# LMCache/LMCache

Hardware: NVIDIA H100
Metric: kv_encode_decode_raw_GBps (higher is better)
Workload: dtype f32->u8 (bf16 KV)

## Files before the change

lmcache_b200/csrc/ac_core.cuh:

```cuda
#pragma once
#include <stdint.h>

#if defined(__CUDACC__)
#define B2_HD __host__ __device__ __forceinline__
#else
#define B2_HD inline
#endif

namespace b200kv {

constexpr int kLp = 33;
constexpr int kMaxSym = 31;
constexpr int kGroup = 256;

B2_HD uint32_t f2u(float f) {
#if defined(__CUDA_ARCH__)
    return __float_as_uint(f);
#else
    union { float f; uint32_t u; } v; v.f = f; return v.u;
#endif
}
B2_HD float u2f(uint32_t u) {
#if defined(__CUDA_ARCH__)
    return __uint_as_float(u);
// ... 599 lines not shown
    const int64_t NL = 2 * (int64_t)L;
    lo.ngroups = (t + kGroup - 1) / kGroup;
    lo.off_cdf = 64;
    if (compact) {
        lo.off_maxes = align16(lo.off_cdf + NL);
        lo.off_lengths = align16(lo.off_maxes + NL * t * 2);
        lo.off_payload = align16(lo.off_lengths + (int64_t)lo.ngroups * NL * C);
    } else {
        lo.off_maxes = align16(lo.off_cdf + NL * C * kLp * 2);
        lo.off_lengths = align16(lo.off_maxes + NL * t * 2);
        lo.off_payload = align16(lo.off_lengths + (int64_t)lo.ngroups * NL * C * 4);
    }
    return lo;
}

constexpr int kHdrMax = 36;
B2_HD int hdr_mask_bytes(int nb) { return (nb + 7) >> 3; }
B2_HD uint32_t hdr_len(uint32_t mask, int nb) {
#if defined(__CUDA_ARCH__)
    const uint32_t nz = (uint32_t)__popc(mask);
#else
    uint32_t nz = 0;
    for (uint32_t m = mask; m; m &= m - 1u) ++nz;
#endif
    const uint32_t h = (uint32_t)hdr_mask_bytes(nb) + (nz ? nz - 1u : 0u);
    return h + (h & 1u);
}
inline uint32_t hdr_write_host(uint8_t* dst, const uint32_t* cnt, int nb) {
    uint32_t mask = 0;
    for (int i = 0; i < nb; ++i) mask |= (cnt[i] ? 1u : 0u) << i;
// ... 12 lines not shown
```

lmcache_b200/csrc/codec.cu:

```cuda
#include <cuda_bf16.h>
#include <cuda_fp16.h>
#include <cuda_runtime.h>
#include <stdint.h>
#include <stdlib.h>
#include <string.h>

#include "ac_core.cuh"
#include "common.cuh"

namespace b200kv {

constexpr int CT = 128;
constexpr int SPW = 6;
constexpr int SYMW = 43;
constexpr int PAIRW = 33;
constexpr int TEMPW_FUSED = 40;
constexpr int TEMPW_SPLIT = 132;
constexpr int TEMPW_FUSED_RANS = 48;
constexpr int CODER_AC = 0, CODER_RANS = 1;
constexpr int CODER_RANS_COMPACT = 2;
constexpr int kHdrRowWords = 8;
constexpr int TEMPW_FUSED_RANS_HDR = TEMPW_FUSED_RANS + kHdrRowWords;

struct EncParams {
// ... 11 lines not shown
    uint64_t* sizes_out;
    uint32_t* temp;
    uint32_t* rstate;
    uint32_t* tile_tot;
    unsigned long long* totals;
    unsigned int* err;
    int32_t lb, nlay;
    uint8_t* arena;
    int64_t arena_bytes;
    unsigned long long* chunk_base;
    unsigned long long* cursor;
    unsigned int* fail_from;
    unsigned long long* ptotal;
    int64_t* seg;
    int32_t layers_left;
};

__device__ __forceinline__ int launch_plane(const EncParams& P, int local) {
    return local + (local < P.nlay ? P.lb : P.L - P.nlay + P.lb);
}

template <class Prm>
__device__ __forceinline__ Layout layout_of(const Prm& P, int t) {
    return make_layout(P.L, P.C, t, P.compact);
}

__device__ __forceinline__ uint32_t load_len(const uint8_t* sec, int64_t idx, bool compact) {
    return compact ? 2u * (uint32_t)sec[idx] : (uint32_t)reinterpret_cast<const int32_t*>(sec)[idx];
}
__device__ __forceinline__ void store_len(uint8_t* sec, int64_t idx, uint32_t len, bool compact) {
    if (compact) sec[idx] = (uint8_t)(len >> 1);
// ... 36 lines not shown
    if (nb > 16) m |= (uint32_t)*reinterpret_cast<const uint16_t*>(p + 2) << 16;
    if (nb <= 8) m &= 0xffu;
    return nb >= 32 ? m : m & ((1u << nb) - 1u);
}

__device__ __forceinline__ int chunk_tokens_of(const EncParams& P, int j) {
    return j == P.n_chunks - 1 ? P.last_chunk_tokens : P.chunk_tokens;
}

template <bool PAGED>
__device__ __forceinline__ int64_t tok_row(const int64_t* slot_map, int64_t tok) {
    if constexpr (PAGED) return __ldg(slot_map + tok);
    else return tok;
}

template <bool VEC, bool PAGED>
__global__ void __launch_bounds__(256) absmax_kernel(EncParams P, int64_t total_tokens) {
    const int64_t warp = (blockIdx.x * (int64_t)blockDim.x + threadIdx.x) >> 5;
    const int lane = threadIdx.x & 31;
    const int64_t nrows = (int64_t)2 * P.nlay * total_tokens;
    if (warp >= nrows) return;
    const int nl = launch_plane(P, (int)(warp / total_tokens));
    const int64_t T = warp % total_tokens;
    const uint16_t* row = P.pt.p[nl] + tok_row<PAGED>(P.slot_map, P.tok_begin + T) * P.sT;
    uint32_t m = 0;
    if (VEC) {
        const int vec_per_head = P.D >> 3;
        const int nvec = P.H * vec_per_head;
        for (int v = lane; v < nvec; v += 32) {
            const int h = v / vec_per_head, dv = v - h * vec_per_head;
            const uint4 q = __ldg(reinterpret_cast<const uint4*>(row + (int64_t)h * P.sH + dv * 8));
            const uint32_t w[4] = {q.x, q.y, q.z, q.w};
#pragma unroll
            for (int k = 0; k < 4; ++k) {
                const uint32_t a = w[k] & 0x7fff7fffu;
                m = max(m, max(a & 0xffffu, a >> 16));
            }
        }
    } else {
        for (int c = lane; c < P.C; c += 32) {
            const int h = c / P.D, d = c - h * P.D;
            m = max(m, (uint32_t)(__ldg(row + (int64_t)h * P.sH + d) & 0x7fffu));
        }
    }
    m = __reduce_max_sync(0xffffffffu, m);
    if (lane == 0) {
        const int j = (int)(T / P.chunk_tokens);
        const int tj = chunk_tokens_of(P, j);
        const Layout lo = layout_of(P, tj);
        uint16_t* maxes = reinterpret_cast<uint16_t*>(P.out + (int64_t)j * P.out_stride + lo.off_maxes);
        maxes[(int64_t)nl * tj + (T - (int64_t)j * P.chunk_tokens)] = (uint16_t)m;
    }
}

__device__ __forceinline__ uint32_t block_excl_scan(uint32_t v, uint32_t* s_warp, uint32_t* total) {
    const int lane = threadIdx.x & 31, wid = threadIdx.x >> 5;
    uint32_t inc = v;
#pragma unroll
    for (int o = 1; o < 32; o <<= 1) {
        uint32_t n = __shfl_up_sync(0xffffffffu, inc, o);
        if (lane >= o) inc += n;
    }
    if (lane == 31) s_warp[wid] = inc;
    __syncthreads();
    uint32_t base = 0, tot = 0;
#pragma unroll
// ... 107 lines not shown
    x = a + start;
    if (r >= freq) x += m;
}

template <bool FUSED, int DT, bool PAGED, int CODER>
__global__ void __launch_bounds__(CT, FUSED ? 7 : 4) encode_kernel(EncParams P) {
    extern __shared__ __align__(128) uint32_t smem[];
    constexpr int ROWS_W = FUSED ? CT * SYMW : 0;
    constexpr int TAB_W = FUSED ? (CT * kLp * 2 + 3) / 4 : CT * PAIRW;
    uint32_t* rows = smem;
    uint32_t* tab = smem + ROWS_W;
    float* fac = reinterpret_cast<float*>(smem + ((ROWS_W + TAB_W + 3) & ~3));
    __shared__ uint32_t s_warp[CT / 32];

    const int tid = threadIdx.x;
    TileId id;
    if (!decode_tile(P, blockIdx.x, &id)) return;
    const int NL = 2 * P.L;
    const int j = id.j, nl = id.nl, ct = id.ct, t = id.t, gt = id.gt;
    const int c = ct * CT + tid;
    const bool active = c < P.C;
    const int ncols = min(CT, P.C - ct * CT);

    uint8_t* cont = P.out + (int64_t)j * P.out_stride;
    const Layout lo = layout_of(P, t);
    const uint16_t* maxes = reinterpret_cast<const uint16_t*>(cont + lo.off_maxes) + (int64_t)nl * t + id.tok0;
    const float maxq = P.pt.maxq[nl];
    const int64_t s1 = P.sT;
    for (int i = tid; i < gt; i += CT)
        fac[i] = FUSED ? quant_factor_safe(maxq, half_to_float(maxes[i], DT)) : quant_factor(maxq, half_to_float(maxes[i], DT));
    if (FUSED) for (int i = gt + tid; i < kGroup + 8; i += CT) fac[i] = 0.0f;

    const int h = active ? c / P.D : 0;
    const int64_t tokabs = P.tok_begin + (int64_t)j * P.chunk_tokens + id.tok0;
    const uint16_t* cbase = P.pt.p[nl] + (int64_t)h * P.sH + (active ? c - h * P.D : 0);
    const uint16_t* src = cbase + (PAGED ? 0 : tokabs * P.sT);
    uint32_t* trow = P.temp + ((int64_t)blockIdx.x * CT + tid) * P.tempw;
    uint32_t cap = (uint32_t)P.tempw;
    asm volatile("" : "+l"(trow), "+r"(cap));
    uint32_t len = 0u, hlen = 0u;

    if (FUSED) {
        uint32_t* myrow = rows + tid * SYMW;
        uint16_t* cdfr = reinterpret_cast<uint16_t*>(tab);
        uint16_t* crow = cdfr + tid * kLp;
        uint16_t* hist = crow;
#pragma unroll
        for (int i = 0; i < kLp; ++i) crow[i] = 0;
        if (!PAGED) {
            const int lines_per_tok = (ncols * 2 + 127) >> 7;
            const uint16_t* tile0 = P.pt.p[nl] + (P.tok_begin + (int64_t)j * P.chunk_tokens + id.tok0) * P.sT +
                                    (int64_t)((ct * CT) / P.D) * P.sH + ((ct * CT) % P.D);
            if ((ct * CT) / P.D == (ct * CT + ncols - 1) / P.D)
                for (int i = tid; i < gt * lines_per_tok; i += CT) {
                    const int tok = i / lines_per_tok, ln = i - tok * lines_per_tok;
                    asm volatile("prefetch.global.L2 [%0];" ::"l"(tile0 + (int64_t)tok * s1 + ln * 64));
                }
        }
        __syncthreads();
        if (active) {
            constexpr int NB = 2, BT = NB * SPW;
            const int nbatch = (gt + BT - 1) / BT;
            uint16_t xa[BT], xb[BT];
            const uint32_t s1u = (uint32_t)s1;
            const uint32_t two = 2u * (uint32_t)min(P.n_chunks, 1);
            auto load = [&](uint16_t (&x)[BT], int b) {
                const int tk = b * BT;
                if constexpr (PAGED) {
                    const int64_t* sm = P.slot_map + tokabs + tk;
#pragma unroll
                    for (int k = 0; k < BT; ++k) x[k] = tk + k < gt ? __ldg(cbase + __ldg(sm + k) * s1) : (uint16_t)0;
                } else {
                    const uint16_t* q = src + (int64_t)tk * s1;
// ... 55 lines not shown
            uint32_t mask = 0u;
#pragma unroll
            for (int i = 0; i < 32; ++i) mask |= (cnt[i] != 0u ? 1u : 0u) << i;
            const uint32_t wany = __reduce_or_sync(__activemask(), mask);
            CdfAccum2 acc;
            acc.init();
#pragma unroll
            for (uint32_t i = 0; i < 32u; ++i) {
                crow[i] = (uint16_t)acc.value(i);
                if ((wany >> i) & 1u) acc.absorb(fac[cnt[i]]);
            }
            crow[32] = (uint16_t)acc.value(32u);
            if (P.compact) {
                uint32_t w0, w1;
                hlen = build_stream_header(cnt, mask, wany, 2 * ((int)maxq + 1), trow, w0, w1);
                reinterpret_cast<uint2*>(P.rstate)[((int64_t)blockIdx.x * CT + tid) * 2] = make_uint2(w0, w1);
            }
        }
        __syncthreads();
        if (!P.compact) {
            uint16_t* dstc = reinterpret_cast<uint16_t*>(cont + lo.off_cdf) + ((int64_t)nl * P.C + ct * CT) * kLp;
            for (int e = tid; e < ncols * kLp; e += CT) dstc[e] = cdfr[e];
        }
        if (active && CODER == CODER_RANS) {
            uint32_t x = kRansLow;
            const uint16_t* const wend = reinterpret_cast<const uint16_t*>(trow) + 2 * P.tempw;
            int32_t nk = 0;
            const char* const cb = reinterpret_cast<const char*>(crow);
            auto code = [&](uint32_t word, int k) {
                const uint32_t o = (k == 0 ? word << 1 : word >> (5 * k - 1)) & 62u;
                const uint32_t c_lo = *reinterpret_cast<const uint16_t*>(cb + o);
                const uint32_t c_hi = *reinterpret_cast<const uint16_t*>(cb + o + 2);
                rans_put(x, nk, wend, c_lo, c_hi - c_lo);
            };
            int w = (gt - 1) / SPW;
            {
                const uint32_t word = myrow[w];
                for (int k = gt - 1 - w * SPW; k >= 0; --k) code(word, k);
            }
            for (--w; w >= 0; --w) {
                const uint32_t word = myrow[w];
#pragma unroll
                for (int k = SPW - 1; k >= 0; --k) code(word, k);
            }
            if (P.compact) reinterpret_cast<uint2*>(P.rstate)[((int64_t)blockIdx.x * CT + tid) * 2 + 1] = make_uint2(x, hlen);
            else P.rstate[(int64_t)blockIdx.x * CT + tid] = x;
            len = hlen + 4u - 2u * (uint32_t)nk;
        } else if (active) {
            EncState2 st;
            st.init();
            int tk = 0;
            for (int w = 0; tk < gt; ++w) {
                const uint32_t word = myrow[w];
                if (tk + SPW <= gt) {
#pragma unroll
                    for (int k = 0; k < SPW; ++k) {
                        const uint32_t sidx = (word >> (5 * k)) & 31u;
                        const uint32_t c_lo = crow[sidx];
                        enc_symbol2(st, c_lo, (uint32_t)crow[sidx + 1u] - c_lo, trow, cap);
                    }
                    tk += SPW;
// ... 19 lines not shown
#pragma unroll
            for (int i = 0; i < kLp; ++i) cv[i] = prow[i] & 0xffffu;
#pragma unroll
            for (int i = 0; i < 32; ++i) {
                const uint32_t hi = (i == 31) ? 0x10000u : cv[i + 1];
                prow[i] = cv[i] | ((hi - cv[i]) << 16);
            }
            if (CODER == CODER_RANS) {
                uint32_t x = kRansLow;
                const uint16_t* const wend = reinterpret_cast<const uint16_t*>(trow) + 2 * TEMPW_SPLIT;
                int32_t nk = 0;
                for_each_symbol_rev<DT, PAGED, 4>(cbase, P.slot_map, tokabs, s1, gt, fac, maxq, [&](uint32_t q) {
                    const uint32_t pr = prow[q];
                    rans_put(x, nk, wend, pr & 0xffffu, pr >> 16);
                });
                P.rstate[(int64_t)blockIdx.x * CT + tid] = x;
                len = 4u - 2u * (uint32_t)nk;
            } else {
                EncState2 st;
                st.init();
                for_each_symbol<DT, PAGED, 4>(cbase, P.slot_map, tokabs, s1, gt, fac, maxq, [&](uint32_t q) {
                    const uint32_t pr = prow[q];
                    enc_symbol2(st, pr & 0xffffu, pr >> 16, trow, cap);
                });
                len = enc_finish2(st, trow, cap);
                if (st.w > cap) atomicOr(&P.err[j], 1u);
            }
        }
    }

    if (active) store_len(cont + lo.off_lengths, ((int64_t)id.g * NL + nl) * P.C + c, len, P.compact != 0);
    uint32_t tile_total;
    (void)block_excl_scan(len, s_warp, &tile_total);
    if (tid == 0) P.tile_tot[(int64_t)j * P.tiles_full + id.tile_in_chunk] = tile_total;
}

template <int DT, bool PAGED>
__global__ void __launch_bounds__(CT) cdf_kernel(EncParams P) {
    extern __shared__ __align__(128) uint32_t smem[];
    uint32_t* cnts = smem;
    float* fac = reinterpret_cast<float*>(cnts + CT * PAIRW);
    const int tid = threadIdx.x;
    const int NL = 2 * P.L;
    const uint32_t per_chunk = (uint32_t)NL * P.tpp;
    const uint32_t j = blockIdx.x / per_chunk;
    const uint32_t rem = blockIdx.x - j * per_chunk;
    const int nl = (int)(rem / P.tpp);
    const int ct = (int)(rem - (uint32_t)nl * P.tpp);
    const int t = chunk_tokens_of(P, (int)j);
// ... 824 lines not shown
        }
        cudaEventRecord(g_prof_ev[slot][0], stream);
    }
    ~ProfScope() {
        if (!g_prof_on) return;
        cudaEventRecord(g_prof_ev[slot][1], stream);
        g_prof_have[slot] = true;
    }
};

static int enc_tempw(bool fused, int coder, bool compact = false) {
    if (compact) return TEMPW_FUSED_RANS_HDR;
    return fused ? (coder == CODER_RANS ? TEMPW_FUSED_RANS : TEMPW_FUSED) : TEMPW_SPLIT;
}

static size_t enc_ws_layout(int64_t n_tiles_alloc, int n_chunks, int tempw, int coder, bool compact, size_t* off_tot,
                            size_t* off_totals, size_t* off_err, size_t* off_state, size_t* off_temp) {
    size_t o = 0;
    *off_tot = o;    o += (size_t)n_tiles_alloc * 4;  o = (o + 255) & ~(size_t)255;
    *off_totals = o; o += (size_t)n_chunks * 8;       o = (o + 255) & ~(size_t)255;
    *off_err = o;    o += (size_t)n_chunks * 4;       o = (o + 255) & ~(size_t)255;
    *off_state = o;  o += coder == CODER_RANS ? (size_t)n_tiles_alloc * CT * (compact ? 16 : 4) : 0;  o = (o + 255) & ~(size_t)255;
    *off_temp = o;   o += (size_t)n_tiles_alloc * CT * (size_t)tempw * 4;
    return (o + 255) & ~(size_t)255;
}

struct EnclWs { size_t err, ptotal, cbase, state, tot, totals, rstate, temp, bytes; };
static EnclWs encl_ws_layout(int n_chunks, int64_t call_tiles) {
    EnclWs w;
    size_t o = 0;
    auto take = [&](size_t* off, size_t n) { *off = o; o = (o + n + 255) & ~(size_t)255; };
    take(&w.err, (size_t)n_chunks * 4);
    take(&w.ptotal, (size_t)n_chunks * 8);
    take(&w.cbase, (size_t)n_chunks * 8);
    take(&w.state, 16);
    take(&w.tot, (size_t)call_tiles * 4);
    take(&w.totals, (size_t)n_chunks * 8);
    take(&w.rstate, (size_t)call_tiles * CT * 16);
    take(&w.temp, (size_t)call_tiles * CT * TEMPW_FUSED_RANS_HDR * 4);
    w.bytes = o;
    return w;
}

constexpr uint32_t kEncPlanMagic = 0x4e4c5045u;
struct EncPlan {
    uint32_t magic;
    int32_t max_layers;
    uint64_t done;
    EncParams P;
};
static_assert(sizeof(EncPlan) <= sizeof(b200kv_encode_plan_t), "b200kv_encode_plan_t too small");

constexpr size_t kSmemFused = (size_t)(((CT * SYMW + (CT * kLp * 2 + 3) / 4 + 3) & ~3) + kGroup + 8) * 4;
constexpr int kStageRans = 12 * 1024;

static int launch_absmax(const EncParams& P, const b200kv_kv_desc* kv, int64_t total_tokens, cudaStream_t stream) {
    bool vec = (kv->D % 8 == 0) && (kv->sT % 8 == 0) && (kv->sH % 8 == 0);
    for (int nl = 0; nl < 2 * P.L && vec; ++nl) vec = (reinterpret_cast<uintptr_t>(P.pt.p[nl]) & 15) == 0;
    const bool paged = P.slot_map != nullptr;
    const int64_t rows = 2 * (int64_t)P.nlay * total_tokens;
    const int64_t blocks = (rows + 7) / 8;
    B2_REQUIRE(blocks < (1ll << 31), "too many rows in one call");
    if (vec && !paged) absmax_kernel<true, false><<<(unsigned)blocks, 256, 0, stream>>>(P, total_tokens);
    else if (vec) absmax_kernel<true, true><<<(unsigned)blocks, 256, 0, stream>>>(P, total_tokens);
    else if (!paged) absmax_kernel<false, false><<<(unsigned)blocks, 256, 0, stream>>>(P, total_tokens);
    else absmax_kernel<false, true><<<(unsigned)blocks, 256, 0, stream>>>(P, total_tokens);
    B2_CHECK_CUDA(cudaGetLastError());
    return 0;
}

static size_t dec_ws_layout(int64_t tiles_max, int n_chunks, size_t* off_tb) {
    size_t o = ((size_t)n_chunks * sizeof(DecChunk) + 255) & ~(size_t)255;
    *off_tb = o;
// ... 69 lines not shown
                                                                                      stride, out);
    B2_CHECK_CUDA(cudaGetLastError());
    return 0;
}

int64_t b200kv_encode_workspace_bytes(int32_t L, int32_t H, int32_t D, int32_t chunk_tokens, int32_t n_chunks,
                                      int32_t coder) {
    if (L <= 0 || H <= 0 || D <= 0 || chunk_tokens <= 0 || n_chunks <= 0) return -2;
    coder &= 0xff;
    const bool compact = coder == CODER_RANS_COMPACT;
    if (compact) coder = CODER_RANS;
    if (coder != CODER_AC && coder != CODER_RANS) return -2;
    if (compact && chunk_tokens > kGroup) return -2;
    const int64_t G = (chunk_tokens + kGroup - 1) / kGroup;
    const int64_t n_tiles = (int64_t)n_chunks * G * 2 * L * tiles_per_plane(H * D);
    size_t a, b, c, d, e;
    return (int64_t)enc_ws_layout(n_tiles, n_chunks, enc_tempw(chunk_tokens <= kGroup, coder, compact), coder, compact, &a, &b, &c, &d, &e);
}

int64_t b200kv_decode_workspace_bytes(int32_t L, int32_t H, int32_t D, int32_t chunk_tokens, int32_t n_chunks) {
    if (L <= 0 || H <= 0 || D <= 0 || chunk_tokens <= 0 || n_chunks <= 0) return -2;
    const int64_t G = (chunk_tokens + kGroup - 1) / kGroup;
    const int64_t tiles_max = G * 2 * L * tiles_per_plane(H * D);
    size_t a;
    return (int64_t)dec_ws_layout(tiles_max, n_chunks, &a);
}

int b200kv_encode_chunks(const b200kv_kv_desc* kv, int64_t tok_begin, int32_t n_chunks, int32_t chunk_tokens,
                         int32_t last_chunk_tokens, const float* key_bins, const float* value_bins, int32_t coder,
                         void* out, int64_t out_stride, uint64_t* sizes_out, void* workspace, int64_t workspace_bytes,
                         void* stream_) {
    cudaStream_t stream = static_cast<cudaStream_t>(stream_);
// ... 12 lines not shown
    B2_REQUIRE(out != nullptr && (reinterpret_cast<uintptr_t>(out) & 15) == 0 && (out_stride & 15) == 0,
               "out / out_stride must be 16-byte aligned");
    B2_REQUIRE(tok_begin >= 0, "tok_begin must be >= 0");
    P.sT = kv->sT; P.sH = kv->sH; P.tok_begin = tok_begin;
    P.slot_map = kv->slot_map;
    const bool paged = kv->slot_map != nullptr;
    P.L = kv->L; P.H = kv->H; P.D = kv->D; P.C = kv->H * kv->D; P.dtype = kv->dtype;
    P.n_chunks = n_chunks; P.chunk_tokens = chunk_tokens; P.last_chunk_tokens = last_chunk_tokens;
    P.tpp = tiles_per_plane(P.C);
    P.out = static_cast<uint8_t*>(out);
    P.out_stride = out_stride;
    P.sizes_out = sizes_out;
    P.lb = 0; P.nlay = P.L;
    P.arena = nullptr; P.arena_bytes = 0; P.chunk_base = nullptr; P.cursor = nullptr; P.fail_from = nullptr;
    P.ptotal = nullptr; P.seg = nullptr; P.layers_left = 0;
    const Layout lo = make_layout(P.L, P.C, chunk_tokens, P.compact);
    B2_REQUIRE(out_stride >= lo.off_payload + 16, "out_stride smaller than the fixed container sections");

    const int64_t G = lo.ngroups;
    const int64_t per_group = 2 * (int64_t)P.L * P.tpp;
    const int64_t tiles_full = G * per_group;
    const int64_t n_tiles = (int64_t)n_chunks * tiles_full;
    const bool fused = chunk_tokens <= kGroup;
    P.tiles_full = (int32_t)tiles_full;
    P.tempw = enc_tempw(fused, coder, P.compact != 0);
    size_t off_tot, off_totals, off_err, off_state, off_temp;
    const size_t need = enc_ws_layout(n_tiles, n_chunks, P.tempw, coder, P.compact != 0, &off_tot, &off_totals, &off_err, &off_state,
                                      &off_temp);
    B2_REQUIRE(workspace != nullptr && workspace_bytes >= (int64_t)need, "workspace too small");
    B2_REQUIRE(n_tiles < (1ll << 31) && tiles_full < (1ll << 31), "too many tiles in one call");
    uint8_t* ws = static_cast<uint8_t*>(workspace);
    P.tile_tot = reinterpret_cast<uint32_t*>(ws + off_tot);
    P.totals = reinterpret_cast<unsigned long long*>(ws + off_totals);
    P.err = reinterpret_cast<unsigned int*>(ws + off_err);
    P.temp = reinterpret_cast<uint32_t*>(ws + off_temp);
    P.rstate = reinterpret_cast<uint32_t*>(ws + off_state);
    B2_CHECK_CUDA(cudaMemsetAsync(ws, 0, off_state, stream));

    const int64_t total_tokens = (int64_t)(n_chunks - 1) * chunk_tokens + last_chunk_tokens;
    for (int i = 0; i <= kProfFinalize; ++i) g_prof_have[i] = false;
    {
        ProfScope prof(kProfAbsmax, stream);
        if (int rc = launch_absmax(P, kv, total_tokens, stream)) return rc;
    }
    const size_t smem_fused = kSmemFused;
    const size_t smem_split = (size_t)(((CT * PAIRW + 3) & ~3) + kGroup + 4) * 4;
    const size_t smem_cdf = (size_t)(CT * PAIRW + kGroup) * 4;
#define B2_LAUNCH_ENC1(FUSED, DT, PAGED, CODER, SMEM)                                                      \
    do {                                                                                                   \
        B2_CHECK_CUDA(cudaFuncSetAttribute(encode_kernel<FUSED, DT, PAGED, CODER>,                         \
                                           cudaFuncAttributeMaxDynamicSharedMemorySize, (int)(SMEM)));     \
        encode_kernel<FUSED, DT, PAGED, CODER><<<(unsigned)n_tiles, CT, (SMEM), stream>>>(P);              \
    } while (0)
#define B2_LAUNCH_ENC(FUSED, DT, PAGED, SMEM)                                                              \
    do {                                                                                                   \
        if (coder == CODER_RANS) B2_LAUNCH_ENC1(FUSED, DT, PAGED, CODER_RANS, SMEM);                       \
        else B2_LAUNCH_ENC1(FUSED, DT, PAGED, CODER_AC, SMEM);                                             \
    } while (0)
#define B2_LAUNCH_ENC2(FUSED, SMEM)                                                                        \
    do {                                                                                                   \
        if (P.dtype == B200KV_DT_BF16) { if (paged) B2_LAUNCH_ENC(FUSED, 0, true, SMEM); else B2_LAUNCH_ENC(FUSED, 0, false, SMEM); } \
        else { if (paged) B2_LAUNCH_ENC(FUSED, 1, true, SMEM); else B2_LAUNCH_ENC(FUSED, 1, false, SMEM); } \
    } while (0)
    if (fused) {
        ProfScope prof(kProfEncode, stream);
        B2_LAUNCH_ENC2(true, smem_fused);
    } else {
// ... 22 lines not shown
        if (coder == CODER_RANS && !hint_mid) P.stage_bytes = 12 * 1024;
        B2_CHECK_CUDA(cudaFuncSetAttribute(compact_kernel, cudaFuncAttributeMaxDynamicSharedMemorySize, P.stage_bytes));
        enc_scan_kernel<<<(unsigned)n_chunks, 1024, 0, stream>>>(P);
        compact_kernel<<<(unsigned)n_tiles, CT, (size_t)P.stage_bytes, stream>>>(P);
        finalize_kernel<<<(n_chunks + 127) / 128, 128, 0, stream>>>(P);
    }
    B2_CHECK_CUDA(cudaGetLastError());
    return 0;
}

int64_t b200kv_encode_layers_workspace_bytes(int32_t L, int32_t H, int32_t D, int32_t chunk_tokens, int32_t n_chunks,
                                             int32_t max_layers) {
    if (L <= 0 || H <= 0 || D <= 0 || chunk_tokens <= 0 || chunk_tokens > kGroup || n_chunks <= 0 || max_layers <= 0 ||
        max_layers > L)
        return -2;
    return (int64_t)encl_ws_layout(n_chunks, (int64_t)n_chunks * 2 * max_layers * tiles_per_plane(H * D)).bytes;
}

int b200kv_encode_layers_plan(const b200kv_kv_desc* kv, int64_t tok_begin, int32_t n_chunks, int32_t chunk_tokens,
                              int32_t last_chunk_tokens, const float* key_bins, const float* value_bins, int32_t coder,
                              void* arena, int64_t arena_bytes, void* fixed_out, int64_t fixed_stride, int64_t* seg_sizes_out,
                              uint64_t* sizes_out, int32_t max_layers, void* workspace, int64_t workspace_bytes,
                              b200kv_encode_plan_t* plan_out, void* stream_) {
    cudaStream_t stream = static_cast<cudaStream_t>(stream_);
    B2_REQUIRE(plan_out != nullptr, "plan is NULL");
    EncPlan* plan = reinterpret_cast<EncPlan*>(plan_out);
    plan->magic = 0u;
    EncParams& P = plan->P;
    B2_REQUIRE(key_bins && value_bins, "bins are NULL");
    B2_REQUIRE((coder & 0xff) == CODER_RANS_COMPACT,
               "the layer-wise encode writes compact containers only (B200KV_CODER_RANS_COMPACT)");
// ... 12 lines not shown
    P.n_chunks = n_chunks; P.chunk_tokens = chunk_tokens; P.last_chunk_tokens = last_chunk_tokens;
    P.tpp = tiles_per_plane(P.C);
    P.coder = CODER_RANS;
    P.compact = 1;
    P.tempw = TEMPW_FUSED_RANS_HDR;
    P.stage_bytes = kStageRans;
    const Layout lo = make_layout(P.L, P.C, chunk_tokens, 1);
    B2_REQUIRE(fixed_stride >= lo.off_payload, "fixed_stride smaller than the fixed container sections");
    P.out = static_cast<uint8_t*>(fixed_out);
    P.out_stride = fixed_stride;
    P.sizes_out = sizes_out;
    P.arena = static_cast<uint8_t*>(arena);
    P.arena_bytes = arena_bytes;
    P.seg = seg_sizes_out;
    const int64_t call_tiles = (int64_t)n_chunks * 2 * max_layers * P.tpp;
    B2_REQUIRE(call_tiles < (1ll << 31), "too many tiles in one call");
    const EnclWs w = encl_ws_layout(n_chunks, call_tiles);
    B2_REQUIRE(workspace != nullptr && workspace_bytes >= (int64_t)w.bytes, "workspace too small");
    uint8_t* ws = static_cast<uint8_t*>(workspace);
    P.err = reinterpret_cast<unsigned int*>(ws + w.err);
    P.ptotal = reinterpret_cast<unsigned long long*>(ws + w.ptotal);
    P.chunk_base = reinterpret_cast<unsigned long long*>(ws + w.cbase);
    P.cursor = reinterpret_cast<unsigned long long*>(ws + w.state);
    P.fail_from = reinterpret_cast<unsigned int*>(ws + w.state + 8);
    P.tile_tot = reinterpret_cast<uint32_t*>(ws + w.tot);
    P.totals = reinterpret_cast<unsigned long long*>(ws + w.totals);
    P.rstate = reinterpret_cast<uint32_t*>(ws + w.rstate);
    P.temp = reinterpret_cast<uint32_t*>(ws + w.temp);
    B2_CHECK_CUDA(cudaMemsetAsync(ws, 0, w.tot, stream));
    B2_CHECK_CUDA(cudaMemsetAsync(fixed_out, 0, (size_t)fixed_stride * n_chunks, stream));
    encl_init_kernel<<<1, 1, 0, stream>>>(P);
    B2_CHECK_CUDA(cudaGetLastError());
    B2_CHECK_CUDA(cudaFuncSetAttribute(compact_kernel, cudaFuncAttributeMaxDynamicSharedMemorySize, P.stage_bytes));
    plan->max_layers = max_layers;
    plan->done = 0ull;
    plan->magic = kEncPlanMagic;
    return 0;
}

int b200kv_encode_layers(b200kv_encode_plan_t* plan_in, int32_t layer_begin, int32_t layer_end, void* stream_) {
    cudaStream_t stream = static_cast<cudaStream_t>(stream_);
    B2_REQUIRE(plan_in != nullptr, "plan is NULL");
    EncPlan* plan = reinterpret_cast<EncPlan*>(plan_in);
    B2_REQUIRE(plan->magic == kEncPlanMagic, "not a plan made by b200kv_encode_layers_plan");
    EncParams P = plan->P;
    B2_REQUIRE(layer_begin >= 0 && layer_begin < layer_end && layer_end <= P.L, "layer range out of range");
    B2_REQUIRE(layer_end - layer_begin <= plan->max_layers, "more layers than the plan's workspace holds");
    const uint64_t bits = (layer_end - layer_begin == 64 ? ~0ull : ((1ull << (layer_end - layer_begin)) - 1ull)) << layer_begin;
    B2_REQUIRE((plan->done & bits) == 0ull, "a layer of the range was encoded before");
    P.lb = layer_begin;
    P.nlay = layer_end - layer_begin;
    P.layers_left = P.L - __builtin_popcountll(plan->done | bits);
    P.tiles_full = 2 * P.nlay * P.tpp;
    const int64_t n_tiles = (int64_t)P.n_chunks * P.tiles_full;
    const int64_t total_tokens = (int64_t)(P.n_chunks - 1) * P.chunk_tokens + P.last_chunk_tokens;
    b200kv_kv_desc kv{};
    kv.D = P.D; kv.sT = P.sT; kv.sH = P.sH;
    if (int rc = launch_absmax(P, &kv, total_tokens, stream)) return rc;
#define B2_LAUNCH_ENCL(DT, PAGED)                                                                                      \
    do {                                                                                                               \
        B2_CHECK_CUDA(cudaFuncSetAttribute(encode_kernel<true, DT, PAGED, CODER_RANS>,                                 \
                                           cudaFuncAttributeMaxDynamicSharedMemorySize, (int)kSmemFused));             \
        encode_kernel<true, DT, PAGED, CODER_RANS><<<(unsigned)n_tiles, CT, kSmemFused, stream>>>(P);                  \
    } while (0)
    if (P.dtype == B200KV_DT_BF16) { if (P.slot_map) B2_LAUNCH_ENCL(0, true); else B2_LAUNCH_ENCL(0, false); }
    else { if (P.slot_map) B2_LAUNCH_ENCL(1, true); else B2_LAUNCH_ENCL(1, false); }
#undef B2_LAUNCH_ENCL
    B2_CHECK_CUDA(cudaGetLastError());
    enc_scan_kernel<<<(unsigned)P.n_chunks, 1024, 0, stream>>>(P);
    place_kernel<<<1, 1024, 0, stream>>>(P);
    compact_kernel<<<(unsigned)n_tiles, CT, (size_t)P.stage_bytes, stream>>>(P);
    B2_CHECK_CUDA(cudaGetLastError());
    plan->done |= bits;
    return 0;
}

int b200kv_encode_layers_finish(const b200kv_encode_plan_t* plan_in, void* stream_) {
    cudaStream_t stream = static_cast<cudaStream_t>(stream_);
    B2_REQUIRE(plan_in != nullptr, "plan is NULL");
    const EncPlan* plan = reinterpret_cast<const EncPlan*>(plan_in);
    B2_REQUIRE(plan->magic == kEncPlanMagic, "not a plan made by b200kv_encode_layers_plan");
    EncParams P = plan->P;
    const uint64_t all = P.L == 64 ? ~0ull : (1ull << P.L) - 1ull;
// ... 168 lines not shown
```

Before: 376.2.

## Fuse absmax pass into encode kernel via ticket-ordered work items

Removes the separate absmax kernel launch in the fused encode path. The encode kernel now takes dynamic tickets from an atomic counter, and each ticket maps to either an absmax work item (a slice of token rows per plane) or an encode tile. Tiles wait on per-plane ready counters that are published with release/acquire, and absmax items are scheduled ahead of their tiles. The row absmax also gets a batched vectorized loader with 8 loads in flight. The change saves a launch and lets absmax overlap with encoding, at the cost of spin-waiting, extra atomics and more complicated tile indexing.

```diff
diff --git a/lmcache_b200/csrc/ac_core.cuh b/lmcache_b200/csrc/ac_core.cuh
--- a/lmcache_b200/csrc/ac_core.cuh
+++ b/lmcache_b200/csrc/ac_core.cuh
@@ -637,6 +637,43 @@
     return lo;
 }
 
+struct EncItem {
+    uint32_t block;
+    uint32_t idx;
+    bool tile;
+};
+B2_HD EncItem enc_item_of(uint32_t ticket, uint32_t nblk, uint32_t tpp, uint32_t R, uint32_t lead) {
+    EncItem it;
+    const uint32_t head = lead < nblk ? lead : nblk;
+    uint32_t u = ticket;
+    if (u < head * R) {
+        it.tile = false;
+        it.block = u / R;
+        it.idx = u - it.block * R;
+        return it;
+    }
+    u -= head * R;
+    const uint32_t paired = nblk - head, per = tpp + R;
+    if (u < paired * per) {
+        const uint32_t k = u / per, r = u - k * per;
+        it.tile = r < tpp;
+        it.block = it.tile ? k : k + lead;
+        it.idx = it.tile ? r : r - tpp;
+        return it;
+    }
+    u -= paired * per;
+    it.tile = true;
+    it.block = paired + u / tpp;
+    it.idx = u - (it.block - paired) * tpp;
+    return it;
+}
+B2_HD int64_t enc_items_total(int64_t nblk, int64_t tpp, int64_t R) { return nblk * (tpp + R); }
+B2_HD void absmax_item_rows(int chunk_tokens, int t, int R, int idx, int* r0, int* r1) {
+    const int per = (chunk_tokens + R - 1) / R;
+    *r0 = idx * per;
+    *r1 = (*r0 + per < t) ? *r0 + per : t;
+}
+
 constexpr int kHdrMax = 36;
 B2_HD int hdr_mask_bytes(int nb) { return (nb + 7) >> 3; }
 B2_HD uint32_t hdr_len(uint32_t mask, int nb) {
diff --git a/lmcache_b200/csrc/codec.cu b/lmcache_b200/csrc/codec.cu
--- a/lmcache_b200/csrc/codec.cu
+++ b/lmcache_b200/csrc/codec.cu
@@ -49,7 +49,15 @@
     unsigned long long* ptotal;
     int64_t* seg;
     int32_t layers_left;
+    unsigned int* ticket;
+    unsigned int* ready;
+    uint32_t ticket_base;
+    int32_t vec;
 };
+
+constexpr int kAbsmaxItems = 16;
+constexpr int kAbsmaxLead = 12;
+static_assert(kAbsmaxLead >= 1, "a tile's absmax items must have smaller tickets than the tile");
 
 __device__ __forceinline__ int launch_plane(const EncParams& P, int local) {
     return local + (local < P.nlay ? P.lb : P.L - P.nlay + P.lb);
@@ -116,6 +124,62 @@
     else return tok;
 }
 
+template <bool VEC>
+__device__ __forceinline__ uint32_t row_absmax(const EncParams& P, const uint16_t* row, int lane) {
+    uint32_t m = 0;
+    if (VEC) {
+        const int vec_per_head = P.D >> 3;
+        const int nvec = P.H * vec_per_head;
+        for (int v = lane; v < nvec; v += 32) {
+            const int h = v / vec_per_head, dv = v - h * vec_per_head;
+            const uint4 q = __ldg(reinterpret_cast<const uint4*>(row + (int64_t)h * P.sH + dv * 8));
+            const uint32_t w[4] = {q.x, q.y, q.z, q.w};
+#pragma unroll
+            for (int k = 0; k < 4; ++k) {
+                const uint32_t a = w[k] & 0x7fff7fffu;
+                m = max(m, max(a & 0xffffu, a >> 16));
+            }
+        }
+    } else {
+        for (int c = lane; c < P.C; c += 32) {
+            const int h = c / P.D, d = c - h * P.D;
+            m = max(m, (uint32_t)(__ldg(row + (int64_t)h * P.sH + d) & 0x7fffu));
+        }
+    }
+    return __reduce_max_sync(0xffffffffu, m);
+}
+
+__device__ __forceinline__ uint32_t row_absmax_batched(const EncParams& P, const uint16_t* row, int lane) {
+    constexpr int K = 8;
+    const int vec_per_head = P.D >> 3;
+    const int nvec = P.H * vec_per_head;
+    const bool flat = P.sH == P.D;
+    uint32_t m = 0;
+    for (int v0 = lane; v0 < nvec; v0 += 32 * K) {
+        uint4 q[K];
+#pragma unroll
+        for (int k = 0; k < K; ++k) {
+            const int v = v0 + 32 * k;
+            q[k] = make_uint4(0u, 0u, 0u, 0u);
+            if (v < nvec) {
+                const int h = flat ? 0 : v / vec_per_head;
+                const int64_t off = flat ? (int64_t)v * 8 : (int64_t)h * P.sH + (v - h * vec_per_head) * 8;
+                q[k] = __ldg(reinterpret_cast<const uint4*>(row + off));
+            }
+        }
+#pragma unroll
+        for (int k = 0; k < K; ++k) {
+            const uint32_t w[4] = {q[k].x, q[k].y, q[k].z, q[k].w};
+#pragma unroll
+            for (int i = 0; i < 4; ++i) {
+                const uint32_t a = w[i] & 0x7fff7fffu;
+                m = max(m, max(a & 0xffffu, a >> 16));
+            }
+        }
+    }
+    return __reduce_max_sync(0xffffffffu, m);
+}
+
 template <bool VEC, bool PAGED>
 __global__ void __launch_bounds__(256) absmax_kernel(EncParams P, int64_t total_tokens) {
     const int64_t warp = (blockIdx.x * (int64_t)blockDim.x + threadIdx.x) >> 5;
@@ -125,33 +189,46 @@
     const int nl = launch_plane(P, (int)(warp / total_tokens));
     const int64_t T = warp % total_tokens;
     const uint16_t* row = P.pt.p[nl] + tok_row<PAGED>(P.slot_map, P.tok_begin + T) * P.sT;
-    uint32_t m = 0;
-    if (VEC) {
-        const int vec_per_head = P.D >> 3;
-        const int nvec = P.H * vec_per_head;
-        for (int v = lane; v < nvec; v += 32) {
-            const int h = v / vec_per_head, dv = v - h * vec_per_head;
-            const uint4 q = __ldg(reinterpret_cast<const uint4*>(row + (int64_t)h * P.sH + dv * 8));
-            const uint32_t w[4] = {q.x, q.y, q.z, q.w};
-#pragma unroll
-            for (int k = 0; k < 4; ++k) {
-                const uint32_t a = w[k] & 0x7fff7fffu;
-                m = max(m, max(a & 0xffffu, a >> 16));
-            }
-        }
-    } else {
-        for (int c = lane; c < P.C; c += 32) {
-            const int h = c / P.D, d = c - h * P.D;
-            m = max(m, (uint32_t)(__ldg(row + (int64_t)h * P.sH + d) & 0x7fffu));
-        }
-    }
-    m = __reduce_max_sync(0xffffffffu, m);
+    const uint32_t m = row_absmax<VEC>(P, row, lane);
     if (lane == 0) {
         const int j = (int)(T / P.chunk_tokens);
         const int tj = chunk_tokens_of(P, j);
         const Layout lo = layout_of(P, tj);
         uint16_t* maxes = reinterpret_cast<uint16_t*>(P.out + (int64_t)j * P.out_stride + lo.off_maxes);
         maxes[(int64_t)nl * tj + (T - (int64_t)j * P.chunk_tokens)] = (uint16_t)m;
+    }
+}
+
+template <bool PAGED>
+__device__ __forceinline__ void absmax_item(const EncParams& P, uint32_t blk, uint32_t item) {
+    const int NL = 2 * P.L;
+    const int j = (int)(blk / (uint32_t)(2 * P.nlay));
+    const int nl = launch_plane(P, (int)(blk - (uint32_t)j * (2 * P.nlay)));
+    const int t = chunk_tokens_of(P, j);
+    int r0, r1;
+    absmax_item_rows(P.chunk_tokens, t, kAbsmaxItems, (int)item, &r0, &r1);
+    const int lane = threadIdx.x & 31;
+    uint16_t* maxes = reinterpret_cast<uint16_t*>(P.out + (int64_t)j * P.out_stride + layout_of(P, t).off_maxes) + (int64_t)nl * t;
+    const int64_t tok0 = P.tok_begin + (int64_t)j * P.chunk_tokens;
+    for (int r = r0 + (int)(threadIdx.x >> 5); r < r1; r += CT / 32) {
+        const uint16_t* row = P.pt.p[nl] + tok_row<PAGED>(P.slot_map, tok0 + r) * P.sT;
+        const uint32_t m = P.vec ? row_absmax_batched(P, row, lane) : row_absmax<false>(P, row, lane);
+        if (lane == 0) maxes[r] = (uint16_t)m;
+    }
+    __syncthreads();
+    if (threadIdx.x == 0) {
+        __threadfence();
+        atomicAdd(P.ready + (int64_t)j * NL + nl, 1u);
+    }
+}
+
+__device__ __forceinline__ void wait_ready(const unsigned int* ready) {
+    uint32_t v, ns = 32;
+    for (;;) {
+        asm volatile("ld.acquire.gpu.global.u32 %0, [%1];" : "=r"(v) : "l"(ready) : "memory");
+        if (v >= (uint32_t)kAbsmaxItems) break;
+        __nanosleep(ns);
+        ns = min(2u * ns, 1024u);
     }
 }
 
@@ -289,8 +366,22 @@
     __shared__ uint32_t s_warp[CT / 32];
 
     const int tid = threadIdx.x;
+    __shared__ uint32_t s_ticket, s_tile;
+    uint32_t tile = blockIdx.x;
+    if constexpr (FUSED) {
+        if (tid == 0) s_ticket = atomicAdd(P.ticket, 1u) - P.ticket_base;
+        __syncthreads();
+        const EncItem it = enc_item_of(s_ticket, (uint32_t)(P.n_chunks * 2 * P.nlay), (uint32_t)P.tpp, kAbsmaxItems, kAbsmaxLead);
+        if (!it.tile) {
+            absmax_item<PAGED>(P, it.block, it.idx);
+            return;
+        }
+        tile = it.block * (uint32_t)P.tpp + it.idx;
+        if (tid == 0) s_tile = tile;
+    }
+    auto late_tile = [&]() -> uint32_t { return FUSED ? s_tile : blockIdx.x; };
     TileId id;
-    if (!decode_tile(P, blockIdx.x, &id)) return;
+    if (!decode_tile(P, tile, &id)) return;
     const int NL = 2 * P.L;
     const int j = id.j, nl = id.nl, ct = id.ct, t = id.t, gt = id.gt;
     const int c = ct * CT + tid;
@@ -302,26 +393,7 @@
     const uint16_t* maxes = reinterpret_cast<const uint16_t*>(cont + lo.off_maxes) + (int64_t)nl * t + id.tok0;
     const float maxq = P.pt.maxq[nl];
     const int64_t s1 = P.sT;
-    for (int i = tid; i < gt; i += CT)
-        fac[i] = FUSED ? quant_factor_safe(maxq, half_to_float(maxes[i], DT)) : quant_factor(maxq, half_to_float(maxes[i], DT));
-    if (FUSED) for (int i = gt + tid; i < kGroup + 8; i += CT) fac[i] = 0.0f;
-
-    const int h = active ? c / P.D : 0;
-    const int64_t tokabs = P.tok_begin + (int64_t)j * P.chunk_tokens + id.tok0;
-    const uint16_t* cbase = P.pt.p[nl] + (int64_t)h * P.sH + (active ? c - h * P.D : 0);
-    const uint16_t* src = cbase + (PAGED ? 0 : tokabs * P.sT);
-    uint32_t* trow = P.temp + ((int64_t)blockIdx.x * CT + tid) * P.tempw;
-    uint32_t cap = (uint32_t)P.tempw;
-    asm volatile("" : "+l"(trow), "+r"(cap));
-    uint32_t len = 0u, hlen = 0u;
-
     if (FUSED) {
-        uint32_t* myrow = rows + tid * SYMW;
-        uint16_t* cdfr = reinterpret_cast<uint16_t*>(tab);
-        uint16_t* crow = cdfr + tid * kLp;
-        uint16_t* hist = crow;
-#pragma unroll
-        for (int i = 0; i < kLp; ++i) crow[i] = 0;
         if (!PAGED) {
             const int lines_per_tok = (ncols * 2 + 127) >> 7;
             const uint16_t* tile0 = P.pt.p[nl] + (P.tok_begin + (int64_t)j * P.chunk_tokens + id.tok0) * P.sT +
@@ -332,6 +404,30 @@
                     asm volatile("prefetch.global.L2 [%0];" ::"l"(tile0 + (int64_t)tok * s1 + ln * 64));
                 }
         }
+        if (tid == 0) wait_ready(P.ready + (int64_t)j * NL + nl);
+        __syncthreads();
+        for (int i = tid; i < gt; i += CT) fac[i] = quant_factor_safe(maxq, half_to_float(maxes[i], DT));
+        for (int i = gt + tid; i < kGroup + 8; i += CT) fac[i] = 0.0f;
+    } else {
+        for (int i = tid; i < gt; i += CT) fac[i] = quant_factor(maxq, half_to_float(maxes[i], DT));
+    }
+
+    const int h = active ? c / P.D : 0;
+    const int64_t tokabs = P.tok_begin + (int64_t)j * P.chunk_tokens + id.tok0;
+    const uint16_t* cbase = P.pt.p[nl] + (int64_t)h * P.sH + (active ? c - h * P.D : 0);
+    const uint16_t* src = cbase + (PAGED ? 0 : tokabs * P.sT);
+    uint32_t* trow = P.temp + ((int64_t)tile * CT + tid) * P.tempw;
+    uint32_t cap = (uint32_t)P.tempw;
+    asm volatile("" : "+l"(trow), "+r"(cap));
+    uint32_t len = 0u, hlen = 0u;
+
+    if (FUSED) {
+        uint32_t* myrow = rows + tid * SYMW;
+        uint16_t* cdfr = reinterpret_cast<uint16_t*>(tab);
+        uint16_t* crow = cdfr + tid * kLp;
+        uint16_t* hist = crow;
+#pragma unroll
+        for (int i = 0; i < kLp; ++i) crow[i] = 0;
         __syncthreads();
         if (active) {
             constexpr int NB = 2, BT = NB * SPW;
@@ -417,7 +513,7 @@
             if (P.compact) {
                 uint32_t w0, w1;
                 hlen = build_stream_header(cnt, mask, wany, 2 * ((int)maxq + 1), trow, w0, w1);
-                reinterpret_cast<uint2*>(P.rstate)[((int64_t)blockIdx.x * CT + tid) * 2] = make_uint2(w0, w1);
+                reinterpret_cast<uint2*>(P.rstate)[((int64_t)late_tile() * CT + tid) * 2] = make_uint2(w0, w1);
             }
         }
         __syncthreads();
@@ -446,8 +542,8 @@
 #pragma unroll
                 for (int k = SPW - 1; k >= 0; --k) code(word, k);
             }
-            if (P.compact) reinterpret_cast<uint2*>(P.rstate)[((int64_t)blockIdx.x * CT + tid) * 2 + 1] = make_uint2(x, hlen);
-            else P.rstate[(int64_t)blockIdx.x * CT + tid] = x;
+            if (P.compact) reinterpret_cast<uint2*>(P.rstate)[((int64_t)late_tile() * CT + tid) * 2 + 1] = make_uint2(x, hlen);
+            else P.rstate[(int64_t)late_tile() * CT + tid] = x;
             len = hlen + 4u - 2u * (uint32_t)nk;
         } else if (active) {
             EncState2 st;
@@ -497,7 +593,7 @@
                     const uint32_t pr = prow[q];
                     rans_put(x, nk, wend, pr & 0xffffu, pr >> 16);
                 });
-                P.rstate[(int64_t)blockIdx.x * CT + tid] = x;
+                P.rstate[(int64_t)late_tile() * CT + tid] = x;
                 len = 4u - 2u * (uint32_t)nk;
             } else {
                 EncState2 st;
@@ -512,10 +608,14 @@
         }
     }
 
-    if (active) store_len(cont + lo.off_lengths, ((int64_t)id.g * NL + nl) * P.C + c, len, P.compact != 0);
+    const uint32_t tile_end = late_tile();
+    if (FUSED) decode_tile(P, tile_end, &id);
+    if (id.ct * CT + tid < P.C)
+        store_len(P.out + (int64_t)id.j * P.out_stride + layout_of(P, id.t).off_lengths,
+                  ((int64_t)id.g * NL + id.nl) * P.C + id.ct * CT + tid, len, P.compact != 0);
     uint32_t tile_total;
     (void)block_excl_scan(len, s_warp, &tile_total);
-    if (tid == 0) P.tile_tot[(int64_t)j * P.tiles_full + id.tile_in_chunk] = tile_total;
+    if (tid == 0) P.tile_tot[tile_end] = tile_total;
 }
 
 template <int DT, bool PAGED>
@@ -1370,19 +1470,20 @@
     return fused ? (coder == CODER_RANS ? TEMPW_FUSED_RANS : TEMPW_FUSED) : TEMPW_SPLIT;
 }
 
-static size_t enc_ws_layout(int64_t n_tiles_alloc, int n_chunks, int tempw, int coder, bool compact, size_t* off_tot,
-                            size_t* off_totals, size_t* off_err, size_t* off_state, size_t* off_temp) {
+static size_t enc_ws_layout(int64_t n_tiles_alloc, int n_chunks, int L, int tempw, int coder, bool compact, size_t* off_tot,
+                            size_t* off_totals, size_t* off_err, size_t* off_sched, size_t* off_state, size_t* off_temp) {
     size_t o = 0;
     *off_tot = o;    o += (size_t)n_tiles_alloc * 4;  o = (o + 255) & ~(size_t)255;
     *off_totals = o; o += (size_t)n_chunks * 8;       o = (o + 255) & ~(size_t)255;
     *off_err = o;    o += (size_t)n_chunks * 4;       o = (o + 255) & ~(size_t)255;
+    *off_sched = o;  o += (1 + (size_t)n_chunks * 2 * L) * 4;  o = (o + 255) & ~(size_t)255;
     *off_state = o;  o += coder == CODER_RANS ? (size_t)n_tiles_alloc * CT * (compact ? 16 : 4) : 0;  o = (o + 255) & ~(size_t)255;
     *off_temp = o;   o += (size_t)n_tiles_alloc * CT * (size_t)tempw * 4;
     return (o + 255) & ~(size_t)255;
 }
 
-struct EnclWs { size_t err, ptotal, cbase, state, tot, totals, rstate, temp, bytes; };
-static EnclWs encl_ws_layout(int n_chunks, int64_t call_tiles) {
+struct EnclWs { size_t err, ptotal, cbase, state, ready, tot, totals, rstate, temp, bytes; };
+static EnclWs encl_ws_layout(int n_chunks, int L, int64_t call_tiles) {
     EnclWs w;
     size_t o = 0;
     auto take = [&](size_t* off, size_t n) { *off = o; o = (o + n + 255) & ~(size_t)255; };
@@ -1390,6 +1491,7 @@
     take(&w.ptotal, (size_t)n_chunks * 8);
     take(&w.cbase, (size_t)n_chunks * 8);
     take(&w.state, 16);
+    take(&w.ready, (size_t)n_chunks * 2 * L * 4);
     take(&w.tot, (size_t)call_tiles * 4);
     take(&w.totals, (size_t)n_chunks * 8);
     take(&w.rstate, (size_t)call_tiles * CT * 16);
@@ -1410,9 +1512,14 @@
 constexpr size_t kSmemFused = (size_t)(((CT * SYMW + (CT * kLp * 2 + 3) / 4 + 3) & ~3) + kGroup + 8) * 4;
 constexpr int kStageRans = 12 * 1024;
 
-static int launch_absmax(const EncParams& P, const b200kv_kv_desc* kv, int64_t total_tokens, cudaStream_t stream) {
-    bool vec = (kv->D % 8 == 0) && (kv->sT % 8 == 0) && (kv->sH % 8 == 0);
+static bool rows_vec_ok(const EncParams& P) {
+    bool vec = (P.D % 8 == 0) && (P.sT % 8 == 0) && (P.sH % 8 == 0);
     for (int nl = 0; nl < 2 * P.L && vec; ++nl) vec = (reinterpret_cast<uintptr_t>(P.pt.p[nl]) & 15) == 0;
+    return vec;
+}
+
+static int launch_absmax(const EncParams& P, int64_t total_tokens, cudaStream_t stream) {
+    const bool vec = P.vec != 0;
     const bool paged = P.slot_map != nullptr;
     const int64_t rows = 2 * (int64_t)P.nlay * total_tokens;
     const int64_t blocks = (rows + 7) / 8;
@@ -1512,8 +1619,9 @@
     if (compact && chunk_tokens > kGroup) return -2;
     const int64_t G = (chunk_tokens + kGroup - 1) / kGroup;
     const int64_t n_tiles = (int64_t)n_chunks * G * 2 * L * tiles_per_plane(H * D);
-    size_t a, b, c, d, e;
-    return (int64_t)enc_ws_layout(n_tiles, n_chunks, enc_tempw(chunk_tokens <= kGroup, coder, compact), coder, compact, &a, &b, &c, &d, &e);
+    size_t a, b, c, d, e, f;
+    return (int64_t)enc_ws_layout(n_tiles, n_chunks, L, enc_tempw(chunk_tokens <= kGroup, coder, compact), coder, compact, &a, &b, &c,
+                                  &d, &e, &f);
 }
 
 int64_t b200kv_decode_workspace_bytes(int32_t L, int32_t H, int32_t D, int32_t chunk_tokens, int32_t n_chunks) {
@@ -1556,6 +1664,8 @@
     P.lb = 0; P.nlay = P.L;
     P.arena = nullptr; P.arena_bytes = 0; P.chunk_base = nullptr; P.cursor = nullptr; P.fail_from = nullptr;
     P.ptotal = nullptr; P.seg = nullptr; P.layers_left = 0;
+    P.ticket_base = 0u;
+    P.vec = rows_vec_ok(P) ? 1 : 0;
     const Layout lo = make_layout(P.L, P.C, chunk_tokens, P.compact);
     B2_REQUIRE(out_stride >= lo.off_payload + 16, "out_stride smaller than the fixed container sections");
 
@@ -1566,24 +1676,27 @@
     const bool fused = chunk_tokens <= kGroup;
     P.tiles_full = (int32_t)tiles_full;
     P.tempw = enc_tempw(fused, coder, P.compact != 0);
-    size_t off_tot, off_totals, off_err, off_state, off_temp;
-    const size_t need = enc_ws_layout(n_tiles, n_chunks, P.tempw, coder, P.compact != 0, &off_tot, &off_totals, &off_err, &off_state,
-                                      &off_temp);
+    size_t off_tot, off_totals, off_err, off_sched, off_state, off_temp;
+    const size_t need = enc_ws_layout(n_tiles, n_chunks, P.L, P.tempw, coder, P.compact != 0, &off_tot, &off_totals, &off_err,
+                                      &off_sched, &off_state, &off_temp);
     B2_REQUIRE(workspace != nullptr && workspace_bytes >= (int64_t)need, "workspace too small");
-    B2_REQUIRE(n_tiles < (1ll << 31) && tiles_full < (1ll << 31), "too many tiles in one call");
+    const int64_t n_ctas = fused ? enc_items_total((int64_t)n_chunks * 2 * P.L, P.tpp, kAbsmaxItems) : n_tiles;
+    B2_REQUIRE(n_ctas < (1ll << 31) && tiles_full < (1ll << 31), "too many tiles in one call");
     uint8_t* ws = static_cast<uint8_t*>(workspace);
     P.tile_tot = reinterpret_cast<uint32_t*>(ws + off_tot);
     P.totals = reinterpret_cast<unsigned long long*>(ws + off_totals);
     P.err = reinterpret_cast<unsigned int*>(ws + off_err);
+    P.ticket = reinterpret_cast<unsigned int*>(ws + off_sched);
+    P.ready = P.ticket + 1;
     P.temp = reinterpret_cast<uint32_t*>(ws + off_temp);
     P.rstate = reinterpret_cast<uint32_t*>(ws + off_state);
     B2_CHECK_CUDA(cudaMemsetAsync(ws, 0, off_state, stream));
 
     const int64_t total_tokens = (int64_t)(n_chunks - 1) * chunk_tokens + last_chunk_tokens;
     for (int i = 0; i <= kProfFinalize; ++i) g_prof_have[i] = false;
-    {
+    if (!fused) {
         ProfScope prof(kProfAbsmax, stream);
-        if (int rc = launch_absmax(P, kv, total_tokens, stream)) return rc;
+        if (int rc = launch_absmax(P, total_tokens, stream)) return rc;
     }
     const size_t smem_fused = kSmemFused;
     const size_t smem_split = (size_t)(((CT * PAIRW + 3) & ~3) + kGroup + 4) * 4;
@@ -1592,7 +1705,7 @@
     do {                                                                                                   \
         B2_CHECK_CUDA(cudaFuncSetAttribute(encode_kernel<FUSED, DT, PAGED, CODER>,                         \
                                            cudaFuncAttributeMaxDynamicSharedMemorySize, (int)(SMEM)));     \
-        encode_kernel<FUSED, DT, PAGED, CODER><<<(unsigned)n_tiles, CT, (SMEM), stream>>>(P);              \
+        encode_kernel<FUSED, DT, PAGED, CODER><<<(unsigned)n_ctas, CT, (SMEM), stream>>>(P);               \
     } while (0)
 #define B2_LAUNCH_ENC(FUSED, DT, PAGED, SMEM)                                                              \
     do {                                                                                                   \
@@ -1645,7 +1758,7 @@
     if (L <= 0 || H <= 0 || D <= 0 || chunk_tokens <= 0 || chunk_tokens > kGroup || n_chunks <= 0 || max_layers <= 0 ||
         max_layers > L)
         return -2;
-    return (int64_t)encl_ws_layout(n_chunks, (int64_t)n_chunks * 2 * max_layers * tiles_per_plane(H * D)).bytes;
+    return (int64_t)encl_ws_layout(n_chunks, L, (int64_t)n_chunks * 2 * max_layers * tiles_per_plane(H * D)).bytes;
 }
 
 int b200kv_encode_layers_plan(const b200kv_kv_desc* kv, int64_t tok_begin, int32_t n_chunks, int32_t chunk_tokens,
@@ -1688,8 +1801,8 @@
     P.arena_bytes = arena_bytes;
     P.seg = seg_sizes_out;
     const int64_t call_tiles = (int64_t)n_chunks * 2 * max_layers * P.tpp;
-    B2_REQUIRE(call_tiles < (1ll << 31), "too many tiles in one call");
-    const EnclWs w = encl_ws_layout(n_chunks, call_tiles);
+    B2_REQUIRE(enc_items_total((int64_t)n_chunks * 2 * P.L, P.tpp, kAbsmaxItems) < (1ll << 31), "too many tiles in one call");
+    const EnclWs w = encl_ws_layout(n_chunks, P.L, call_tiles);
     B2_REQUIRE(workspace != nullptr && workspace_bytes >= (int64_t)w.bytes, "workspace too small");
     uint8_t* ws = static_cast<uint8_t*>(workspace);
     P.err = reinterpret_cast<unsigned int*>(ws + w.err);
@@ -1697,6 +1810,10 @@
     P.chunk_base = reinterpret_cast<unsigned long long*>(ws + w.cbase);
     P.cursor = reinterpret_cast<unsigned long long*>(ws + w.state);
     P.fail_from = reinterpret_cast<unsigned int*>(ws + w.state + 8);
+    P.ticket = reinterpret_cast<unsigned int*>(ws + w.state + 12);
+    P.ready = reinterpret_cast<unsigned int*>(ws + w.ready);
+    P.ticket_base = 0u;
+    P.vec = rows_vec_ok(P) ? 1 : 0;
     P.tile_tot = reinterpret_cast<uint32_t*>(ws + w.tot);
     P.totals = reinterpret_cast<unsigned long long*>(ws + w.totals);
     P.rstate = reinterpret_cast<uint32_t*>(ws + w.rstate);
@@ -1727,20 +1844,18 @@
     P.layers_left = P.L - __builtin_popcountll(plan->done | bits);
     P.tiles_full = 2 * P.nlay * P.tpp;
     const int64_t n_tiles = (int64_t)P.n_chunks * P.tiles_full;
-    const int64_t total_tokens = (int64_t)(P.n_chunks - 1) * P.chunk_tokens + P.last_chunk_tokens;
-    b200kv_kv_desc kv{};
-    kv.D = P.D; kv.sT = P.sT; kv.sH = P.sH;
-    if (int rc = launch_absmax(P, &kv, total_tokens, stream)) return rc;
+    const int64_t n_ctas = enc_items_total((int64_t)P.n_chunks * 2 * P.nlay, P.tpp, kAbsmaxItems);
 #define B2_LAUNCH_ENCL(DT, PAGED)                                                                                      \
     do {                                                                                                               \
         B2_CHECK_CUDA(cudaFuncSetAttribute(encode_kernel<true, DT, PAGED, CODER_RANS>,                                 \
                                            cudaFuncAttributeMaxDynamicSharedMemorySize, (int)kSmemFused));             \
-        encode_kernel<true, DT, PAGED, CODER_RANS><<<(unsigned)n_tiles, CT, kSmemFused, stream>>>(P);                  \
+        encode_kernel<true, DT, PAGED, CODER_RANS><<<(unsigned)n_ctas, CT, kSmemFused, stream>>>(P);                   \
     } while (0)
     if (P.dtype == B200KV_DT_BF16) { if (P.slot_map) B2_LAUNCH_ENCL(0, true); else B2_LAUNCH_ENCL(0, false); }
     else { if (P.slot_map) B2_LAUNCH_ENCL(1, true); else B2_LAUNCH_ENCL(1, false); }
 #undef B2_LAUNCH_ENCL
     B2_CHECK_CUDA(cudaGetLastError());
+    plan->P.ticket_base += (uint32_t)n_ctas;
     enc_scan_kernel<<<(unsigned)P.n_chunks, 1024, 0, stream>>>(P);
     place_kernel<<<1, 1024, 0, stream>>>(P);
     compact_kernel<<<(unsigned)n_tiles, CT, (size_t)P.stage_bytes, stream>>>(P);
```

New measurement: 380.5, median of 6. 1.01x the previous value.
